# soedinglab/plass

Measured on AMD Instinct MI355X. Metric: read-overlaps/s per assembly iteration, higher is better.
Workload: dtype u8/u64 (integer hash, byte compare; f32 ratios)

## Files before the change

plass_amd/csrc/assemble.hip:

```cpp
#include "common.hpp"
#include "device_utils.hpp"
#include "posterior_class.hpp"
#include "host_util.hpp"
#include <algorithm>
#include <memory>
#include <cstring>

namespace plasship {

struct Item {
    uint32_t target; int32_t score; uint32_t alnLength; float seqId;
    int32_t qStart, qEnd; uint32_t qLen; int32_t dbStart, dbEnd; uint32_t dbLen;
    uint32_t state;
    uint32_t pad;
};

struct AsmArgs {
    SeqView s;
    const uint64_t *qoff; const AlnRec *recs;
    Item *items;
    const uint64_t *arenaOff;
    const uint32_t *leftCap;
    char *arena;
    uint32_t *flags;
    uint32_t *newLen;
    uint64_t *newStart;
    const signed char *mat;
    double lambda, logK, ln2;
    float seqIdThr; uint64_t maxSeqLen; int rescoreMode;
    uint32_t ownLaneMin;
    unsigned long long *stats;
    uint32_t *bigList; uint32_t nBig;
    uint32_t *midList; uint32_t nMid;
    uint32_t *mid32List; uint32_t nMid32;
    uint32_t *smallList; uint32_t nSmall;
    uint32_t *heap;
    const uint32_t *ambKeys; const uint8_t *ambVals; uint32_t ambMask;
    uint32_t *needKeys; uint32_t *needCount; uint32_t needCap;
    uint32_t *redoList; uint32_t *redoCount;
    const uint32_t *queryList; uint32_t nQueryList;
    uint8_t *cmpCache;
    SeqView aa; char *aaArena; const uint64_t *aaArenaOff; const uint32_t *aaLeftCap; uint32_t *aaNewLen; uint64_t *aaNewStart;
};

__device__ __forceinline__ float seqIdThroughText(float f) {
    if (f == 1.0f) return 1.0f;
    const int t = (int) (f * 1000);
    int zeros = 0;
    if ((double) f < 0.10) zeros++;
    if ((double) f < 0.01) zeros++;
    int digits = 1; for (int x = t; x >= 10; x /= 10) digits++;
    double den = 1.0; for (int i = 0; i < digits + zeros; i++) den *= 10.0;
    return (float) ((double) t / den);
}

__device__ __forceinline__ uint64_t loadU64Unaligned(const char *p) { uint64_t w; __builtin_memcpy(&w, p, 8); return w; }
__device__ __forceinline__ void storeU64Unaligned(char *p, uint64_t w) { __builtin_memcpy(p, &w, 8); }
__device__ __forceinline__ void storeTail(char *d, uint64_t v, unsigned r) {
    if (r & 4u) { const uint32_t x = (uint32_t) v; __builtin_memcpy(d, &x, 4); d += 4; v >>= 32; }
    if (r & 2u) { const uint16_t x = (uint16_t) v; __builtin_memcpy(d, &x, 2); d += 2; v >>= 16; }
    if (r & 1u) *d = (char) v;
}
template <int G> __device__ __forceinline__ void copyBytesG(char *dst, const char *src, unsigned n, int gl) {
    for (unsigned i = 8u * (unsigned) gl; i < n; i += 8u * G) {
        const uint64_t w = loadU64Unaligned(src + i);
        if (i + 8 <= n) storeU64Unaligned(dst + i, w);
        else storeTail(dst + i, w, n - i);
    }
}
__device__ __forceinline__ void stageScoreTable(signed char *smat, const signed char *__restrict__ mat, int nThreads) {
    for (int i = threadIdx.x; i < 123 * 123; i += nThreads) smat[i] = i ? mat[i] : (signed char) 0;
}
__device__ __forceinline__ uint64_t byteRangeMask(int lo, int hi) {
    const uint64_t belowHi = hi >= 8 ? ~0ULL : (hi <= 0 ? 0ULL : ((1ULL << (8 * hi)) - 1ULL));
    const uint64_t belowLo = lo >= 8 ? ~0ULL : (lo <= 0 ? 0ULL : ((1ULL << (8 * lo)) - 1ULL));
    return belowHi & ~belowLo;
}
__device__ __forceinline__ int zeroBytes(uint64_t x, uint64_t mask) {
    const uint64_t lo7 = 0x7F7F7F7F7F7F7F7FULL;
    return __popcll(~(((x & lo7) + lo7) | x | lo7) & mask);
}
template <int G> __device__ __forceinline__ void scoreColumnsG(const char *q, const char *t, unsigned len, const signed char *smat, int gl,
                                                               unsigned &first, unsigned &last, int &s, int &ids) {
    const unsigned p0 = 8u * (unsigned) gl;
    uint64_t qw = 0, tw = 0;
// ... 23 lines not shown
__device__ __forceinline__ void scoreColumnsSerial(const char *q, const char *t, unsigned len, const signed char *smat,
                                                   unsigned &first, unsigned &last, int &s, int &ids) {
    const char q0 = q[0], t0 = t[0], qe = q[len - 1], te = t[len - 1];
    uint64_t qw[4], tw[4];
    __builtin_memcpy(qw, q, 32); __builtin_memcpy(tw, t, 32);
    first = (q0 == '*' || t0 == '*') ? 1u : 0u;
    last = len - 1;
    if (last > 0 && (qe == '*' || te == '*')) last--;
    for (unsigned p = 0; p < len; p += 32) {
        if (p) { __builtin_memcpy(qw, q + p, 32); __builtin_memcpy(tw, t + p, 32); }
#pragma unroll
        for (unsigned k = 0; k < 4; k++) {
            const int lo = (int) first - (int) (p + 8 * k), hi = (int) last - (int) (p + 8 * k);
            uint64_t qv = qw[k], tv = tw[k];
            if (lo <= 0 && hi >= 8) ids += zeroBytes(qw[k] ^ tw[k], ~0ULL);
            else {
                const uint64_t m = byteRangeMask(lo, hi + 1);
                ids += zeroBytes(qw[k] ^ tw[k], byteRangeMask(lo, hi));
                qv = qw[k] & m; tv = tw[k] & m;
            }
#pragma unroll
            for (unsigned j = 0; j < 8; j++) {
                const unsigned a = (unsigned) (qv >> (8 * j)) & 0xFFu, b = (unsigned) (tv >> (8 * j)) & 0xFFu;
                s += (int) smat[a * 123 + b];
            }
        }
    }
}

struct Rescored { int startPos, endPos; unsigned score, diagonalLen; int idExcl; };
__device__ __forceinline__ Rescored rescoreOnDiagonal(const char *q, unsigned qLen, const char *t, unsigned tLen, int diagonal,
                                                      const signed char *smat) {
    Rescored r; r.startPos = -1; r.endPos = -1; r.score = 0; r.diagonalLen = 0; r.idExcl = 0;
    const unsigned dist = (unsigned) abs(diagonal);
    unsigned qo, to, len;
    if (diagonal >= 0 && dist < qLen) { qo = dist; to = 0; len = min(tLen, qLen - dist); }
    else if (diagonal < 0 && dist < tLen) { qo = 0; to = dist; len = min(tLen - dist, qLen); }
    else return r;
    r.diagonalLen = len;
    if (len == 0) return r;
    unsigned first, last;
    int s = 0, ids = 0;
    scoreColumnsG<64>(q + qo, t + to, len, smat, laneId(), first, last, s, ids);
    s = waveReduceSum(s); ids = waveReduceSum(ids);
    r.score = (unsigned) max(s, 0); r.startPos = (int) first; r.endPos = (int) last; r.idExcl = ids;
    return r;
}

__device__ __forceinline__ void waveMemSync() {
    __builtin_amdgcn_fence(__ATOMIC_RELEASE, "workgroup");
    __builtin_amdgcn_fence(__ATOMIC_ACQUIRE, "workgroup");
}
__global__ __launch_bounds__(256) void assembleBigKernel(AsmArgs a) {
    __shared__ signed char smat[123 * 123 + 7];
    stageScoreTable(smat, a.mat, 256);
    __syncthreads();
    const int lane = threadIdx.x & 63;
    unsigned long long nExt = 0, nResc = 0, nRescRes = 0, nAln = 0, nQRes = 0;
    for (uint32_t w = blockIdx.x * 4 + (threadIdx.x >> 6); w < a.nBig; w += gridDim.x * 4) {
        const uint32_t id = a.bigList[w];
        const uint64_t h0 = a.qoff[id], h1 = a.qoff[id + 1];
        const uint32_t h = (uint32_t) (h1 - h0);
        if (h == 0) continue;
        const uint64_t aoff = a.arenaOff[id];
        if (a.arenaOff[id + 1] == aoff) continue;
        Item *it = a.items + h0;
        const char *orig = a.s.data + seqOff(a.s, id);
        unsigned querySeqLen = seqLen(a.s, id);
        nAln += h; nQRes += querySeqLen;
        for (uint32_t i = lane; i < h; i += 64) {
            const AlnRec r = a.recs[h0 + i];
            Item x;
            x.target = r.target;
            const int aq = (r.qStart == -1) ? 0 : r.qStart, ad = (r.dbStart == -1) ? 0 : r.dbStart;
            x.alnLength = (uint32_t) (max(abs(r.qEnd - aq), abs(r.dbEnd - ad)) + 1);
            const int rawScore = (int) (fma((double) r.bitScore, a.ln2, a.logK) / a.lambda + 0.5);
            const float scorePerCol = (float) rawScore / (float) ((double) x.alnLength + 0.5);
            const float sid = r.fromText ? r.seqId : seqIdThroughText(r.seqId);
            const float alnLen = (float) x.alnLength;
            const float ids = sid * alnLen;
            x.seqId = (float) ((double) ids / ((double) alnLen + 0.5));
            x.score = (int) (scorePerCol * 100);
            x.qStart = r.qStart; x.qEnd = r.qEnd; x.qLen = (uint32_t) r.qLen; x.dbStart = r.dbStart; x.dbEnd = r.dbEnd; x.dbLen = (uint32_t) r.dbLen;
            x.state = r.accepted ? 0u : 2u; x.pad = 0;
            it[i] = x;
        }
        char *buf = a.arena + aoff;
        uint64_t curStart = a.leftCap[id];
        copyBytesG<64>(buf + curStart, orig, querySeqLen, lane);
        uint64_t curLen = querySeqLen;
        waveMemSync();
        bool couldExtend = false;
        uint32_t inQueue = h;
        while (inQueue > 0) {
            unsigned leftOff = 0, rightOff = 0;
            bool brokeOut = false;
            unsigned long long bestR = 0, bestL = 0; uint32_t idxR = 0xFFFFFFFFu, idxL = 0xFFFFFFFFu;
            for (uint32_t i = lane; i < h; i += 64) {
                Item x = it[i];
                if (x.state == 1) { it[i].state = 2; continue; }
                if (x.state != 0) continue;
                const unsigned long long key = ((unsigned long long) ((uint32_t) x.score ^ 0x80000000u) << 32) | (unsigned long long) x.alnLength;
                const bool notBoth = !(x.dbStart == 0 && x.qStart == 0);
                const bool rightStart = x.dbStart == 0 && (x.dbEnd != (int) x.dbLen - 1);
                const bool leftStart = x.qStart == 0 && (x.qEnd != (int) x.qLen - 1);
                if (!((rightStart || leftStart) && notBoth) || x.target == id) continue;
                const unsigned tLen = seqLen(a.s, x.target);
                if (x.dbStart == 0) {
                    const unsigned fragR = tLen - ((unsigned) x.dbEnd + 1);
                    if (fragR > 0 && (unsigned) x.qEnd == (querySeqLen - 1) && (key > bestR || (key == bestR && x.target < it[idxR].target))) { bestR = key; idxR = i; }
                } else if (x.qStart == 0) {
                    if (x.dbStart > 0 && (unsigned) x.dbEnd == (tLen - 1) && (key > bestL || (key == bestL && x.target < it[idxL].target))) { bestL = key; idxL = i; }
                }
            }
            uint32_t tgtR = idxR != 0xFFFFFFFFu ? it[idxR].target : 0xFFFFFFFFu, tgtL = idxL != 0xFFFFFFFFu ? it[idxL].target : 0xFFFFFFFFu;
#pragma unroll
            for (int o = 32; o > 0; o >>= 1) {
                const unsigned long long okR = __shfl_xor(bestR, o, 64), okL = __shfl_xor(bestL, o, 64);
                const uint32_t oiR = __shfl_xor(idxR, o, 64), oiL = __shfl_xor(idxL, o, 64), otR = __shfl_xor(tgtR, o, 64), otL = __shfl_xor(tgtL, o, 64);
                if (oiR != 0xFFFFFFFFu && (idxR == 0xFFFFFFFFu || okR > bestR || (okR == bestR && otR < tgtR))) { bestR = okR; idxR = oiR; tgtR = otR; }
                if (oiL != 0xFFFFFFFFu && (idxL == 0xFFFFFFFFu || okL > bestL || (okL == bestL && otL < tgtL))) { bestL = okL; idxL = oiL; tgtL = otL; }
            }
            const bool haveR = idxR != 0xFFFFFFFFu, haveL = idxL != 0xFFFFFFFFu;
            const bool rFirst = haveR && (!haveL || bestR > bestL || (bestR == bestL && tgtR < tgtL));
            waveMemSync();
            auto extendRight = [&]() {
                const Item x = it[idxR];
                const char *tSeq = a.s.data + seqOff(a.s, x.target);
                const unsigned tLen = seqLen(a.s, x.target), dbEnd = (unsigned) x.dbEnd, fragLen = tLen - (dbEnd + 1);
                copyBytesG<64>(buf + curStart + curLen, tSeq + dbEnd + 1, fragLen, lane);
                curLen += fragLen; rightOff += fragLen;
                if (lane == 0) atomicOr(&a.flags[x.target], 0x80u);
            };
            if (rFirst) extendRight();
            if (haveL) {
                const Item x = it[idxL];
                const unsigned fragLen = (unsigned) x.dbStart;
                if (curLen + fragLen >= a.maxSeqLen) brokeOut = true;
                else {
                    const char *tSeq = a.s.data + seqOff(a.s, x.target);
                    curStart -= fragLen;
                    copyBytesG<64>(buf + curStart, tSeq, fragLen, lane);
                    curLen += fragLen; leftOff += fragLen;
                    if (lane == 0) atomicOr(&a.flags[x.target], 0x80u);
                }
            }
            if (haveR && !rFirst && !brokeOut) extendRight();
            waveMemSync();
            uint32_t still = 0;
// ... 11 lines not shown
                const bool rightStart = x.dbStart == 0 && (x.dbEnd != (int) x.dbLen - 1);
                const bool leftStart = x.qStart == 0 && (x.qEnd != (int) x.qLen - 1);
                if (!used && (rightStart || leftStart) && notBoth && x.target != id) {
                    const unsigned tLen = seqLen(a.s, x.target);
                    if (x.dbStart == 0) { if ((tLen - ((unsigned) x.dbEnd + 1)) > rightOff && (unsigned) x.qEnd == (querySeqLen - 1) && rightOff > 0) st = 1; }
                    else if (x.qStart == 0) { if (x.dbStart > (int) leftOff && (unsigned) x.dbEnd == (tLen - 1) && leftOff > 0) st = 1; }
                }
                it[i].state = st;
            }
            inQueue = (uint32_t) waveReduceSum((int) still);
            waveMemSync();
            if (leftOff > 0 || rightOff > 0) couldExtend = true;
            if (brokeOut && inQueue > 0) break;
            querySeqLen = (unsigned) curLen;
            const char *qs = buf + curStart;
            waveMemSync();
            for (uint32_t i = lane; i < h; i += 64) {
                Item x = it[i];
                if (x.state != 1) continue;
                const char *tSeq = a.s.data + seqOff(a.s, x.target);
                const unsigned tLen = seqLen(a.s, x.target);
                const int diag = (int) ((unsigned) x.qStart + leftOff) - x.dbStart;
                const unsigned dist = (unsigned) abs(diag);
                unsigned qo = 0, to = 0, len = 0; bool hit = true;
                if (diag >= 0 && dist < querySeqLen) { qo = dist; to = 0; len = min(tLen, querySeqLen - dist); }
                else if (diag < 0 && dist < tLen) { qo = 0; to = dist; len = min(tLen - dist, querySeqLen); }
                else hit = false;
                unsigned first = 0, last = 0; int sc = 0, ids = 0; int startPos = -1, endPos = -1;
                if (hit && len > 0) { scoreColumnsSerial(qs + qo, tSeq + to, len, smat, first, last, sc, ids); startPos = (int) first; endPos = (int) last; }
                const unsigned score = (unsigned) max(sc, 0);
                nResc++; nRescRes += hit ? len : 0;
                int qS, qE, dS, dE;
                if (diag >= 0) { qS = startPos + (int) dist; qE = endPos + (int) dist; dS = startPos; dE = endPos; }
                else { qS = startPos; qE = endPos; dS = startPos + (int) dist; dE = endPos + (int) dist; }
                const float seqId = (float) ids / ((float) qE - (float) qS);
                x.seqId = seqId; x.qLen = querySeqLen; x.dbLen = tLen; x.alnLength = hit ? len : 0u;
                const float spc = (float) score / (float) ((double) x.alnLength + 0.5);
                x.score = (int) (spc * 100);
                x.qStart = qS; x.qEnd = qE; x.dbStart = dS; x.dbEnd = dE;
                x.state = (seqId >= a.seqIdThr) ? 0u : 2u;
                it[i] = x;
            }
            waveMemSync();
            {
                uint32_t c = 0;
                for (uint32_t i = lane; i < h; i += 64) c += (it[i].state == 0) ? 1u : 0u;
                inQueue = (uint32_t) waveReduceSum((int) c);
            }
        }
        if (couldExtend) {
            if (lane == 0) { atomicOr(&a.flags[id], 0x20u); a.newLen[id] = (uint32_t) curLen; a.newStart[id] = aoff + curStart; }
            nExt++;
        }
        waveMemSync();
    }
    nResc = waveReduceSumU64(nResc); nRescRes = waveReduceSumU64(nRescRes);
    if (lane == 0) {
        if (nExt) atomicAdd(&a.stats[0], nExt); if (nResc) atomicAdd(&a.stats[1], nResc); if (nRescRes) atomicAdd(&a.stats[2], nRescRes);
        if (nAln) { atomicAdd(&a.stats[9], nAln); atomicAdd(&a.stats[10], nQRes); atomicAdd(&a.stats[11], nRescRes); }
    }
}

__device__ __forceinline__ char nuclRevN(char c) {
    switch (c & ~0x20) {
        case 'A': return 'T';
        case 'C': case 'M': case 'Y': case 'H': return 'G';
        case 'T': case 'U': case 'W': return 'A';
        case 'G': case 'K': case 'B': case 'D': case 'V': case 'R': case 'S': return 'C';
        default: return 'N';
    }
}
constexpr unsigned CMP_LEN = 512, CMP_MM = 8;
struct NuclCmp { const AsmArgs *a; bool abort; };
__device__ __forceinline__ uint32_t ambHash(uint32_t a1, uint32_t b1, uint32_t a2, uint32_t b2) {
    return (a1 * 0x9E3779B1u) ^ (b1 * 0x85EBCA77u) ^ (a2 * 0xC2B2AE3Du) ^ (b2 * 0x27D4EB2Fu);
}
__device__ __attribute__((noinline)) int nuclPosteriorClassDev(unsigned alpha1, unsigned beta1, unsigned alpha2, unsigned beta2, const AsmArgs *ap) {
    const double p = nuclPosteriorP(alpha1, beta1, alpha2, beta2);
    int cls = (p < 0.45) ? 0 : ((p > 0.55) ? 1 : 2);
    const double AMB_EPS = nuclPosteriorBand(alpha1, beta1, alpha2, beta2);
    if (fabs(p - 0.45) < AMB_EPS || fabs(p - 0.55) < AMB_EPS) {
        const AsmArgs &a = *ap;
        if (a.ambMask) {
            uint32_t slot = ambHash(alpha1, beta1, alpha2, beta2) & a.ambMask;
            for (;;) {
                const uint32_t *k = a.ambKeys + 4 * (size_t) slot;
                if (k[0] == 0) break;
                if (k[0] == alpha1 && k[1] == beta1 && k[2] == alpha2 && k[3] == beta2) return (int) a.ambVals[slot];
                slot = (slot + 1) & a.ambMask;
            }
        }
        const uint32_t w = atomicAdd(a.needCount, 1u);
        if (w < a.needCap) { uint32_t *k = a.needKeys + 4 * (size_t) w; k[0] = alpha1; k[1] = beta1; k[2] = alpha2; k[3] = beta2; }
        return -1;
    }
    return cls;
}
__device__ __forceinline__ bool nuclLess(const Item &r1, const Item &r2, NuclCmp &c) {
    if (c.abort) return false;
    const unsigned mm1 = (unsigned) ((double) ((1.0f - r1.seqId) * (float) r1.alnLength) + 0.5);
    const unsigned mm2 = (unsigned) ((double) ((1.0f - r2.seqId) * (float) r2.alnLength) + 0.5);
    const bool cacheable = c.a->cmpCache && mm1 < CMP_MM && mm2 < CMP_MM && r1.alnLength < CMP_LEN && r2.alnLength < CMP_LEN;
    const size_t cidx = cacheable ? ((((size_t) r1.alnLength * CMP_MM + mm1) * CMP_LEN + r2.alnLength) * CMP_MM + mm2) : 0;
    int cls = cacheable ? (int) c.a->cmpCache[cidx] - 1 : -1;
    if (cls < 0) {
        cls = nuclPosteriorClassDev(mm1 + 1, r1.alnLength - mm1 + 1, mm2 + 1, r2.alnLength - mm2 + 1, c.a);
        if (cls < 0) { c.abort = true; return false; }
// ... 1132 lines not shown
    }
    const unsigned gridN = std::min<uint32_t>((N + 255) / 256 + 1, 8192);
    hipLaunchKernelGGL(extMarkKernel, dim3(gridN), dim3(256), 0, st, N, dFlags, dNewLen, guided ? dAaNewLen : (const uint32_t *) nullptr, dKeep.as<uint32_t>(), dBytes.as<uint64_t>(),
                       guided ? dAaBytes.as<uint64_t>() : (uint64_t *) nullptr);
    if (exclusiveScanU32(st, dKeep.as<uint32_t>(), dPos.as<uint64_t>(), N, dTmp, tmpBytes) || exclusiveScanU64(st, dBytes.as<uint64_t>(), dOff.as<uint64_t>(), N, dTmp, tmpBytes) ||
        (guided && exclusiveScanU64(st, dAaBytes.as<uint64_t>(), dAaOff.as<uint64_t>(), N, dTmp, tmpBytes))) { setError("plasship_assemble: scan failed"); return PLASSHIP_ERR_DEVICE; }
    uint64_t nExt = 0, extBytes = 0, aaExtBytes = 0;
    PH_CHECK(hipMemcpyAsync(&nExt, dPos.as<uint64_t>() + N, 8, hipMemcpyDeviceToHost, st));
    PH_CHECK(hipMemcpyAsync(&extBytes, dOff.as<uint64_t>() + N, 8, hipMemcpyDeviceToHost, st));
    if (guided) PH_CHECK(hipMemcpyAsync(&aaExtBytes, dAaOff.as<uint64_t>() + N, 8, hipMemcpyDeviceToHost, st));
    PH_CHECK(plasship::streamSync(st));
    DevBuf dMeta, dPacked, dAaPacked;
    if (dMeta.alloc(std::max<uint64_t>(nExt, 1) * sizeof(ExtMeta)) != hipSuccess || dPacked.alloc(extBytes + 64) != hipSuccess || (guided && dAaPacked.alloc(aaExtBytes + 64) != hipSuccess)) {
        setError("plasship_assemble: out of device memory"); return PLASSHIP_ERR_DEVICE;
    }
    if (N) hipLaunchKernelGGL(extPackKernel, dim3(std::min<uint32_t>((N + 15) / 16, (uint32_t) ctx->numCU * 16)), dim3(256), 0, st, N, dKeep.as<uint32_t>(), dPos.as<uint64_t>(), dOff.as<uint64_t>(),
                              guided ? dAaOff.as<uint64_t>() : (const uint64_t *) nullptr, dNewLen, dNewStart, dArena, dAaNewLen, dAaNewStart, dAaArena,
                              dMeta.as<ExtMeta>(), dPacked.as<char>(), guided ? dAaPacked.as<char>() : (char *) nullptr);
    PH_TRACE(st, "assemble: packed the extended sequences");
    DevBuf gMeta; std::vector<uint64_t> rb(W), rbMeta(W), rbSeq(W), rbAa(W);
    uint64_t M = 0;
    {
        const uint64_t mine[3] = {nExt, extBytes, aaExtBytes}; std::vector<uint64_t> all(3 * (size_t) W);
        const int rc0 = commAllgatherHost(ctx, mine, all.data(), 24); if (rc0) return rc0;
        for (int r = 0; r < W; r++) { M += all[3 * (size_t) r]; rbMeta[r] = all[3 * (size_t) r] * sizeof(ExtMeta); rbSeq[r] = all[3 * (size_t) r + 1]; rbAa[r] = all[3 * (size_t) r + 2]; }
    }
    int rc = commAllgathervBytesKnown(ctx, dMeta.p, nExt * sizeof(ExtMeta), gMeta, rbMeta); if (rc) return rc;
    rc = commAllgathervBytesKnown(ctx, dPacked.p, extBytes, gathered, rbSeq); if (rc) return rc;
    if (guided) { rc = commAllgathervBytesKnown(ctx, dAaPacked.p, aaExtBytes, gatheredAa, rbAa); if (rc) return rc; }
    PH_TRACE(st, "assemble: gathered the extended sequences");
    DevBuf dLens, dStart, dAaLens, dAaStart, dTmp2; const size_t tmp2Bytes = exclusiveScanTmpBytes(M + 2);
    if (dLens.alloc((M + 1) * 8) != hipSuccess || dStart.alloc((M + 2) * 8) != hipSuccess || dTmp2.alloc(tmp2Bytes) != hipSuccess ||
        (guided && (dAaLens.alloc((M + 1) * 8) != hipSuccess || dAaStart.alloc((M + 2) * 8) != hipSuccess))) { setError("plasship_assemble: out of device memory"); return PLASSHIP_ERR_DEVICE; }
    if (M) {
        const unsigned gridM = (unsigned) std::min<uint64_t>((M + 255) / 256, 8192);
        hipLaunchKernelGGL(extLensKernel, dim3(gridM), dim3(256), 0, st, gMeta.as<ExtMeta>(), M, dLens.as<uint64_t>(), guided ? dAaLens.as<uint64_t>() : (uint64_t *) nullptr);
        if (exclusiveScanU64(st, dLens.as<uint64_t>(), dStart.as<uint64_t>(), M, dTmp2.p, tmp2Bytes) ||
            (guided && exclusiveScanU64(st, dAaLens.as<uint64_t>(), dAaStart.as<uint64_t>(), M, dTmp2.p, tmp2Bytes))) { setError("plasship_assemble: scan failed"); return PLASSHIP_ERR_DEVICE; }
        hipLaunchKernelGGL(extMergeKernel, dim3(gridM), dim3(256), 0, st, gMeta.as<ExtMeta>(), M, dStart.as<uint64_t>(), guided ? dAaStart.as<uint64_t>() : (const uint64_t *) nullptr,
                           dFlags, dNewLen, dNewStart, dAaNewLen, dAaNewStart);
    }
    PH_TRACE(st, "assemble: merged the extended sequences");
    if (!keepTarget) {
        DevBuf gFlags;
        rc = commAllgathervBytes(ctx, dFlags, (uint64_t) N * 4, gFlags, rb); if (rc) return rc;
        if (N) hipLaunchKernelGGL(orFlagsKernel, dim3(gridN), dim3(256), 0, st, gFlags.as<uint32_t>(), N, W, dFlags);
        PH_CHECK(plasship::streamSync(st));
    }
    PH_CHECK(plasship::streamSync(st));
    PH_CHECK(hipGetLastError());
    return PLASSHIP_OK;
}

static int assembleImpl(plasship_ctx *ctx, const plasship_seqdb *db, const plasship_seqdb *aaDb, const plasship_alns *al,
                        const plasship_assemble_params *par, plasship_seqdb **out, plasship_seqdb **outAa, plasship_assemble_stats *stats) {
    const bool guided = aaDb != nullptr;
    const bool nucl = db->dbtype == PLASSHIP_DBTYPE_NUCLEOTIDES;
    if (!nucl && db->dbtype != PLASSHIP_DBTYPE_AMINO_ACIDS) { setError("plasship_assemble: the sequence DB is neither amino acids nor nucleotides"); return PLASSHIP_ERR_ARG; }
    if (par->rescore_mode != 3) { setError("plasship_assemble: only --rescore-mode 3"); return PLASSHIP_ERR_UNSUPPORTED; }
    if (al->nQueries != db->n) { setError("plasship_assemble: alignment list does not belong to the DB"); return PLASSHIP_ERR_ARG; }
    PH_ENTER(ctx);
    hipStream_t st = ctx->stream;
    const uint32_t N = (uint32_t) db->n;
    if (nucl) { const int rcS = finishSelfAlns(ctx, al); if (rcS) return rcS; }
    const uint64_t nLines = al->nSlots;
    DevBuf dLeftCap, dBytes, dArenaOff, dTmp, dItems, dFlags, dNewLen, dNewStart, dMat, dStats, dArena;
    const size_t tmpBytes = exclusiveScanTmpBytes((size_t) N + 2);
    if (dLeftCap.alloc(((size_t) N + 1) * 4) != hipSuccess || dBytes.alloc(((size_t) N + 1) * 8) != hipSuccess || dArenaOff.alloc(((size_t) N + 2) * 8) != hipSuccess ||
        dTmp.alloc(tmpBytes) != hipSuccess || dItems.alloc(std::max<uint64_t>(nLines, 1) * sizeof(Item)) != hipSuccess || dFlags.alloc(((size_t) N + 1) * 4) != hipSuccess ||
        dNewLen.alloc(((size_t) N + 1) * 4) != hipSuccess || dNewStart.alloc(((size_t) N + 1) * 8) != hipSuccess || dMat.alloc(123 * 123) != hipSuccess || dStats.alloc(128) != hipSuccess) {
        setError("plasship_assemble: out of device memory"); return PLASSHIP_ERR_DEVICE;
    }
    PH_CHECK(hipMemsetAsync(dFlags.p, 0, ((size_t) N + 1) * 4, st));
    PH_CHECK(hipMemsetAsync(dNewLen.p, 0, ((size_t) N + 1) * 4, st));
    PH_CHECK(hipMemsetAsync(dStats.p, 0, 128, st));
    PH_CHECK(hipMemcpyAsync(dMat.p, asciiSubMat(nucl), 123 * 123, hipMemcpyHostToDevice, st));
    { const int rcOL = ensureOffLen(ctx, db); if (rcOL) return rcOL; }
    const SeqView sv = db->view();
    PH_CHECK(hipEventRecord(ctx->ev[0], st));
    DevBuf dBigList, dMidList, dMid32List, dSmallList, dTierA, dTierB, dPosA, dPosB, dAaLeftCap, dAaBytes, dAaArenaOff, dAaArena, dAaNewLen, dAaNewStart;
    if (guided && (dAaLeftCap.alloc(((size_t) N + 1) * 4) != hipSuccess || dAaBytes.alloc(((size_t) N + 1) * 8) != hipSuccess || dAaArenaOff.alloc(((size_t) N + 2) * 8) != hipSuccess ||
                   dAaNewLen.alloc(((size_t) N + 1) * 4) != hipSuccess || dAaNewStart.alloc(((size_t) N + 1) * 8) != hipSuccess)) { setError("plasship_assemble: out of device memory"); return PLASSHIP_ERR_DEVICE; }
    if (guided) PH_CHECK(hipMemsetAsync(dAaNewLen.p, 0, ((size_t) N + 1) * 4, st));
    if (dBigList.alloc(((size_t) N + 1) * 4) != hipSuccess || dMidList.alloc(((size_t) N + 1) * 4) != hipSuccess || dMid32List.alloc(((size_t) N + 1) * 4) != hipSuccess ||
        dSmallList.alloc(((size_t) N + 1) * 4) != hipSuccess || dTierA.alloc(((size_t) N + 1) * 8) != hipSuccess || dTierB.alloc(((size_t) N + 1) * 8) != hipSuccess ||
        dPosA.alloc(((size_t) N + 2) * 8) != hipSuccess || dPosB.alloc(((size_t) N + 2) * 8) != hipSuccess) { setError("plasship_assemble: out of device memory"); return PLASSHIP_ERR_DEVICE; }
    DevBuf dQSum, dQSumAa, dQCan;
    if (dQSum.alloc(((size_t) N + 1) * 8) != hipSuccess || dQCan.alloc(((size_t) N + 1) * 4) != hipSuccess || (guided && dQSumAa.alloc(((size_t) N + 1) * 8) != hipSuccess)) { setError("plasship_assemble: out of device memory"); return PLASSHIP_ERR_DEVICE; }
    PH_CHECK(hipMemsetAsync(dQSum.p, 0, ((size_t) N + 1) * 8, st));
    PH_CHECK(hipMemsetAsync(dQCan.p, 0, ((size_t) N + 1) * 4, st));
    if (guided) PH_CHECK(hipMemsetAsync(dQSumAa.p, 0, ((size_t) N + 1) * 8, st));
    if (nLines) hipLaunchKernelGGL(arenaSumKernel, dim3((unsigned) std::min<uint64_t>((nLines + 255) / 256, (uint64_t) ctx->numCU * 32)), dim3(256), 0, st, al->d_recs.as<AlnRec>(), (uint64_t) nLines,
                                       (uint64_t) par->max_seq_len, dQSum.as<unsigned long long>(), guided ? dQSumAa.as<unsigned long long>() : (unsigned long long *) nullptr, dQCan.as<uint32_t>(),
                                       (nucl && !guided) ? 1 : 0);
    if (N) hipLaunchKernelGGL(arenaSizeKernel, dim3(std::min<uint32_t>((N + 255) / 256, 8192)), dim3(256), 0, st, sv, al->d_qoff.as<uint64_t>(), (const unsigned long long *) dQSum.as<unsigned long long>(),
                              (const unsigned long long *) dQSumAa.as<unsigned long long>(), (const uint32_t *) dQCan.as<uint32_t>(), dLeftCap.as<uint32_t>(), dBytes.as<uint64_t>(), nucl ? 1 : 0, (uint64_t) tuneInt("NUCL_THREAD_BYTES", 1 << 30),
                              dTierA.as<uint64_t>(), dTierB.as<uint64_t>(),
                              guided ? aaDb->d_len.as<uint32_t>() : (const uint32_t *) nullptr, dAaLeftCap.as<uint32_t>(), guided ? dAaBytes.as<uint64_t>() : (uint64_t *) nullptr);
    if (guided && exclusiveScanU64(st, dAaBytes.as<uint64_t>(), dAaArenaOff.as<uint64_t>(), N, dTmp.p, tmpBytes)) { setError("plasship_assemble: scan failed"); return PLASSHIP_ERR_DEVICE; }
    if (exclusiveScanU64(st, dTierA.as<uint64_t>(), dPosA.as<uint64_t>(), N, dTmp.p, tmpBytes) || exclusiveScanU64(st, dTierB.as<uint64_t>(), dPosB.as<uint64_t>(), N, dTmp.p, tmpBytes)) {
        setError("plasship_assemble: scan failed"); return PLASSHIP_ERR_DEVICE;
    }
    if (N) hipLaunchKernelGGL(listKernel, dim3(std::min<uint32_t>((N + 255) / 256, 8192)), dim3(256), 0, st, N, dTierA.as<uint64_t>(), dTierB.as<uint64_t>(), dPosA.as<uint64_t>(), dPosB.as<uint64_t>(),
                              dSmallList.as<uint32_t>(), dMid32List.as<uint32_t>(), dMidList.as<uint32_t>(), dBigList.as<uint32_t>());
    if (exclusiveScanU64(st, dBytes.as<uint64_t>(), dArenaOff.as<uint64_t>(), N, dTmp.p, tmpBytes)) { setError("plasship_assemble: scan failed"); return PLASSHIP_ERR_DEVICE; }
    uint64_t arenaBytes = 0, aaArenaBytes = 0;
// ... 58 lines not shown
                if (cnts[0]) {
                    a.queryList = dSmallList.as<uint32_t>(); a.nQueryList = cnts[0];
                    if (tuneInt("NUCL_CLASSES", 1) == 1) {
                        DevBuf dCls;
                        if (dCls.alloc(2 * NW_CLASSES * 4) != hipSuccess) { setError("plasship_assemble: out of device memory"); return PLASSHIP_ERR_DEVICE; }
                        PH_CHECK(hipMemsetAsync(dCls.p, 0, 2 * NW_CLASSES * 4, st));
                        const unsigned g = std::min<uint32_t>((cnts[0] + 255) / 256, (uint32_t) ctx->numCU * 8);
                        hipLaunchKernelGGL(nuclClassCountKernel, dim3(g), dim3(256), 0, st, (const uint32_t *) dSmallList.as<uint32_t>(), cnts[0], (const uint64_t *) dBytes.as<uint64_t>(), dCls.as<uint32_t>());
                        hipLaunchKernelGGL(nuclClassScatterKernel, dim3(g), dim3(256), 0, st, (const uint32_t *) dSmallList.as<uint32_t>(), cnts[0], (const uint64_t *) dBytes.as<uint64_t>(), dCls.as<uint32_t>(),
                                           dMidList.as<uint32_t>());
                        a.queryList = dMidList.as<uint32_t>();
                    }
                    const uint32_t grid = std::min<uint32_t>((cnts[0] + NT_BLOCK - 1) / NT_BLOCK, (uint32_t) ctx->numCU * 8);
                    if (guided) hipLaunchKernelGGL(assembleNuclThreadKernel<true>, dim3(grid), dim3(NT_BLOCK), 0, st, a);
                    else hipLaunchKernelGGL(assembleNuclThreadKernel<false>, dim3(grid), dim3(NT_BLOCK), 0, st, a);
                }
                launchWave(dMid32List.as<uint32_t>(), cnts[1]);
            } else launchWave(dRedo[(pass + 1) & 1].as<uint32_t>(), nWork);
            uint32_t cnt[2] = {0, 0};
            PH_CHECK(hipMemcpyAsync(cnt, dCnt.p, 8, hipMemcpyDeviceToHost, st));
            PH_CHECK(plasship::streamSync(st));
            PH_CHECK(hipGetLastError());
            nWork = cnt[1];
            if (nWork == 0) break;
            const uint32_t nNeed = std::min(cnt[0], needCap);
            if (nNeed == 0) { setError("plasship_assemble: queries aborted without a missing comparator tuple"); return PLASSHIP_ERR_DEVICE; }
            std::vector<uint32_t> need((size_t) nNeed * 4);
            PH_COPY_SYNC(ctx->stream, need.data(), dNeed.p, need.size() * 4, hipMemcpyDeviceToHost);
            const int rc = ambTableInsert(ctx, need.data(), nNeed);
            if (rc != PLASSHIP_OK) return rc;
        }
        PH_CHECK(hipEventRecord(ctx->ev[3], st));
        for (int e = 4; e <= 7; e++) PH_CHECK(hipEventRecord(ctx->ev[e], st));
    } else {
    const int w16 = tuneInt("ASM16", 5), w64 = tuneInt("ASM64", 4);
    const uint32_t gx = (uint32_t) std::max(1, tuneInt("ASM_GRIDX", 1));
    const dim3 g16(std::min<uint32_t>((a.nSmall + 15) / 16, (uint32_t) ctx->numCU * (uint32_t) w16 * gx)), g64(std::min<uint32_t>((a.nMid + 3) / 4, (uint32_t) ctx->numCU * (uint32_t) w64 * gx));
    PH_CHECK(hipEventRecord(ctx->ev[2], st));
    if (a.nSmall) {
        if (w16 == 6) hipLaunchKernelGGL((assembleGroupKernel<16, 6>), g16, dim3(256), 0, st, a);
        else if (w16 == 5) hipLaunchKernelGGL((assembleGroupKernel<16, 5>), g16, dim3(256), 0, st, a);
        else hipLaunchKernelGGL((assembleGroupKernel<16, 4>), g16, dim3(256), 0, st, a);
    }
    PH_CHECK(hipEventRecord(ctx->ev[3], st));
    PH_CHECK(hipEventRecord(ctx->ev[4], st));
    if (a.nMid32) hipLaunchKernelGGL((assembleGroupKernel<32, 5>), dim3(std::min<uint32_t>((a.nMid32 + 7) / 8, (uint32_t) ctx->numCU * 5u * gx)), dim3(256), 0, st, a);
    if (a.nMid) {
        if (w64 == 5) hipLaunchKernelGGL((assembleGroupKernel<64, 5>), g64, dim3(256), 0, st, a);
        else if (w64 == 4) hipLaunchKernelGGL((assembleGroupKernel<64, 4>), g64, dim3(256), 0, st, a);
        else hipLaunchKernelGGL((assembleGroupKernel<64, 3>), g64, dim3(256), 0, st, a);
    }
    PH_CHECK(hipEventRecord(ctx->ev[5], st));
    PH_CHECK(hipEventRecord(ctx->ev[6], st));
    if (a.nBig) hipLaunchKernelGGL(assembleBigKernel, dim3(std::min<uint32_t>((a.nBig + 3) / 4, (uint32_t) ctx->numCU * (uint32_t) tuneInt("ASMBIG", 4))), dim3(256), 0, st, a);
    PH_CHECK(hipEventRecord(ctx->ev[7], st));
    }
    PH_TRACE(st, "assemble: extension kernels");
    plasship_seqdb *o = nullptr, *oAa = nullptr;
    unsigned long long hs[16] = {0};
    DevBuf dGathered, dGatheredAa;
    const char *arenaP = dArena.as<char>(), *aaArenaP = dAaArena.as<char>();
    if (commOf(ctx)) {
        const int rc = mergeExtended(ctx, N, guided, par->keep_target, dFlags.as<uint32_t>(), dNewLen.as<uint32_t>(), dNewStart.as<uint64_t>(), dArena.as<char>(),
                                     dAaNewLen.as<uint32_t>(), dAaNewStart.as<uint64_t>(), dAaArena.as<char>(), dTmp.p, tmpBytes, dGathered, dGatheredAa);
        if (rc != PLASSHIP_OK) return rc;
        arenaP = dGathered.as<char>(); aaArenaP = dGatheredAa.as<char>();
    }
    int rcOut = buildOutputDB(ctx, db, dFlags.as<uint32_t>(), dNewLen.as<uint32_t>(), dNewStart.as<uint64_t>(), arenaP, par->keep_target, dTmp.p, tmpBytes, &o,
                              dStats.p, hs, 128, guided ? (hipEvent_t) nullptr : ctx->ev[1], guided);
    if (rcOut != PLASSHIP_OK) return rcOut;
    std::unique_ptr<plasship_seqdb> holdO(o), holdAa;
    if (guided) {
        rcOut = buildOutputDB(ctx, aaDb, dFlags.as<uint32_t>(), dAaNewLen.as<uint32_t>(), dAaNewStart.as<uint64_t>(), aaArenaP, par->keep_target, dTmp.p, tmpBytes, &oAa,
                              nullptr, nullptr, 0, nullptr, true);
        if (rcOut != PLASSHIP_OK) return rcOut;
        holdAa.reset(oAa);
    }
    if (guided) { PH_CHECK(hipEventRecord(ctx->ev[1], st)); PH_CHECK(plasship::streamSync(st)); }
    if (hs[12]) { setError("plasship_guided_assemble: an alignment asks for a protein fragment the twin does not have (coordinates are not codon aligned)"); return PLASSHIP_ERR_ARG; }
    if (stats) {
        stats->n_extended = hs[0]; stats->n_rescored = hs[1]; stats->out_residues = o->residues;
        float ms = 0; (void) hipEventElapsedTime(&ms, ctx->ev[0], ctx->ev[1]); stats->ms_kernel = ms;
        float sum = 0;
        for (int t = 0; t < 3; t++) {
            ms = 0; (void) hipEventElapsedTime(&ms, ctx->ev[2 + 2 * t], ctx->ev[3 + 2 * t]); stats->ms_tier_kernel[t] = ms; sum += ms;
            stats->tier_alignments[t] = hs[3 + 3 * t]; stats->tier_query_residues[t] = hs[4 + 3 * t]; stats->tier_rescored_residues[t] = hs[5 + 3 * t];
        }
        stats->ms_assemble_kernel = sum;
        stats->n_alignments = al->nLines; stats->rescored_residues = hs[2];
        stats->db_appended_bytes = o->buildAppendedBytes; stats->db_copied_bytes = o->buildCopiedBytes;
    }
    *out = holdO.release();
    if (guided) *outAa = holdAa.release();
    return PLASSHIP_OK;
}

extern "C" int plasship_assemble(plasship_ctx *ctx, const plasship_seqdb *db, const plasship_alns *al,
                                 const plasship_assemble_params *par, plasship_seqdb **out, plasship_assemble_stats *stats) {
    if (!ctx || !db || !al || !par || !out) { setError("plasship_assemble: bad argument"); return PLASSHIP_ERR_ARG; }
    return commFinish(ctx, assembleImpl(ctx, db, nullptr, al, par, out, nullptr, stats));
}

extern "C" int plasship_guided_assemble(plasship_ctx *ctx, const plasship_seqdb *nucl_db, const plasship_seqdb *aa_db, const plasship_alns *al,
                                        const plasship_assemble_params *par, plasship_seqdb **out_nucl, plasship_seqdb **out_aa,
                                        plasship_assemble_stats *stats) {
    if (!ctx || !nucl_db || !aa_db || !al || !par || !out_nucl || !out_aa) { setError("plasship_guided_assemble: bad argument"); return PLASSHIP_ERR_ARG; }
    if (nucl_db->dbtype != PLASSHIP_DBTYPE_NUCLEOTIDES || aa_db->dbtype != PLASSHIP_DBTYPE_AMINO_ACIDS) { setError("plasship_guided_assemble: needs a nucleotide DB and its protein twin DB"); return PLASSHIP_ERR_ARG; }
    if (nucl_db->n != aa_db->n) { setError("plasship_guided_assemble: the two DBs differ in size"); return PLASSHIP_ERR_ARG; }
// ... 7 lines not shown
```

Baseline: 707.4 million.

## Add LDS-resident compacting queue kernels for big-query assembly with overflow fallback

```diff
diff --git a/plass_amd/csrc/assemble.hip b/plass_amd/csrc/assemble.hip
--- a/plass_amd/csrc/assemble.hip
+++ b/plass_amd/csrc/assemble.hip
@@ -31,6 +31,10 @@
     uint32_t ownLaneMin;
     unsigned long long *stats;
     uint32_t *bigList; uint32_t nBig;
+    const uint32_t *bigCount;
+    uint32_t *overList; uint32_t *overCount;
+    uint32_t queueCap;
+    uint32_t *dbgRounds; uint32_t *dbgCycles;
     uint32_t *midList; uint32_t nMid;
     uint32_t *mid32List; uint32_t nMid32;
     uint32_t *smallList; uint32_t nSmall;
@@ -160,12 +164,14 @@
     __builtin_amdgcn_fence(__ATOMIC_ACQUIRE, "workgroup");
 }
 __global__ __launch_bounds__(256) void assembleBigKernel(AsmArgs a) {
+    const uint32_t nBig = a.bigCount ? *a.bigCount : a.nBig;
+    if (blockIdx.x * 4 >= nBig) return;
     __shared__ signed char smat[123 * 123 + 7];
     stageScoreTable(smat, a.mat, 256);
     __syncthreads();
     const int lane = threadIdx.x & 63;
     unsigned long long nExt = 0, nResc = 0, nRescRes = 0, nAln = 0, nQRes = 0;
-    for (uint32_t w = blockIdx.x * 4 + (threadIdx.x >> 6); w < a.nBig; w += gridDim.x * 4) {
+    for (uint32_t w = blockIdx.x * 4 + (threadIdx.x >> 6); w < nBig; w += gridDim.x * 4) {
         const uint32_t id = a.bigList[w];
         const uint64_t h0 = a.qoff[id], h1 = a.qoff[id + 1];
         const uint32_t h = (uint32_t) (h1 - h0);
@@ -176,6 +182,7 @@
         const char *orig = a.s.data + seqOff(a.s, id);
         unsigned querySeqLen = seqLen(a.s, id);
         nAln += h; nQRes += querySeqLen;
+        const uint64_t t0 = a.dbgRounds ? (uint64_t) clock64() : 0; uint32_t rounds = 0;
         for (uint32_t i = lane; i < h; i += 64) {
             const AlnRec r = a.recs[h0 + i];
             Item x;
@@ -203,6 +210,7 @@
         while (inQueue > 0) {
             unsigned leftOff = 0, rightOff = 0;
             bool brokeOut = false;
+            rounds++;
             unsigned long long bestR = 0, bestL = 0; uint32_t idxR = 0xFFFFFFFFu, idxL = 0xFFFFFFFFu;
             for (uint32_t i = lane; i < h; i += 64) {
                 Item x = it[i];
@@ -320,7 +328,213 @@
             if (lane == 0) { atomicOr(&a.flags[id], 0x20u); a.newLen[id] = (uint32_t) curLen; a.newStart[id] = aoff + curStart; }
             nExt++;
         }
+        if (a.dbgRounds && lane == 0) { a.dbgRounds[id] = rounds | (couldExtend ? 0x80000000u : 0u); a.dbgCycles[id] = (uint32_t) min<uint64_t>((uint64_t) clock64() - t0, 0xFFFFFFFFull); }
         waveMemSync();
+    }
+    nResc = waveReduceSumU64(nResc); nRescRes = waveReduceSumU64(nRescRes);
+    if (lane == 0) {
+        if (nExt) atomicAdd(&a.stats[0], nExt); if (nResc) atomicAdd(&a.stats[1], nResc); if (nRescRes) atomicAdd(&a.stats[2], nRescRes);
+        if (nAln) { atomicAdd(&a.stats[9], nAln); atomicAdd(&a.stats[10], nQRes); atomicAdd(&a.stats[11], nRescRes); }
+    }
+}
+
+constexpr uint32_t ASMQ_CAP1 = 128, ASMQ_CAP = 256;
+template <int CAP> struct QueueLds {
+    unsigned long long key[CAP];
+    uint64_t offLen[CAP];
+    uint32_t target[CAP], qLen[CAP], dbLen[CAP];
+    int32_t qStart[CAP], qEnd[CAP], dbStart[CAP], dbEnd[CAP];
+};
+struct QItem { unsigned long long key; uint64_t offLen; uint32_t target, qLen, dbLen; int32_t qStart, qEnd, dbStart, dbEnd; };
+template <int CAP> __device__ __forceinline__ QItem qLoad(const QueueLds<CAP> &q, uint32_t i) {
+    QItem x;
+    x.key = q.key[i]; x.offLen = q.offLen[i]; x.target = q.target[i]; x.qLen = q.qLen[i]; x.dbLen = q.dbLen[i];
+    x.qStart = q.qStart[i]; x.qEnd = q.qEnd[i]; x.dbStart = q.dbStart[i]; x.dbEnd = q.dbEnd[i];
+    return x;
+}
+template <int CAP> __device__ __forceinline__ void qStore(QueueLds<CAP> &q, uint32_t i, const QItem &x) {
+    q.key[i] = x.key; q.offLen[i] = x.offLen; q.target[i] = x.target; q.qLen[i] = x.qLen; q.dbLen[i] = x.dbLen;
+    q.qStart[i] = x.qStart; q.qEnd[i] = x.qEnd; q.dbStart[i] = x.dbStart; q.dbEnd[i] = x.dbEnd;
+}
+template <int CAP> __device__ __forceinline__ uint32_t qCompact(QueueLds<CAP> &q, uint32_t base, bool keep, const QItem &x) {
+    const unsigned long long m = __ballot(keep);
+    if (keep) qStore(q, base + (uint32_t) __builtin_amdgcn_mbcnt_hi((uint32_t) (m >> 32), __builtin_amdgcn_mbcnt_lo((uint32_t) m, 0u)), x);
+    return (uint32_t) __popcll(m);
+}
+__device__ __forceinline__ void queueFence() { __builtin_amdgcn_fence(__ATOMIC_ACQ_REL, "wavefront"); __builtin_amdgcn_wave_barrier(); }
+__device__ __forceinline__ unsigned long long queueKey(int score, uint32_t alnLength) {
+    return ((unsigned long long) ((uint32_t) score ^ 0x80000000u) << 32) | (unsigned long long) alnLength;
+}
+
+template <int CAP, int WPE>
+__global__ __launch_bounds__(256) __attribute__((amdgpu_waves_per_eu(WPE, WPE))) void assembleQueueKernel(AsmArgs a) {
+    const uint32_t nBig = a.bigCount ? *a.bigCount : a.nBig;
+    if (blockIdx.x * 4 >= nBig) return;
+    __shared__ signed char smat[123 * 123 + 7];
+    __shared__ QueueLds<CAP> queues[4];
+    stageScoreTable(smat, a.mat, 256);
+    __syncthreads();
+    const int lane = threadIdx.x & 63;
+    QueueLds<CAP> &q = queues[threadIdx.x >> 6];
+    unsigned long long nExt = 0, nResc = 0, nRescRes = 0, nAln = 0, nQRes = 0;
+    for (uint32_t w = blockIdx.x * 4 + (threadIdx.x >> 6); w < nBig; w += gridDim.x * 4) {
+        const uint32_t id = a.bigList[w];
+        const uint64_t h0 = a.qoff[id], h1 = a.qoff[id + 1];
+        const uint32_t h = (uint32_t) (h1 - h0);
+        if (h == 0) continue;
+        if (h > CAP || h > a.queueCap) {
+            if (lane == 0) a.overList[atomicAdd(a.overCount, 1u)] = id;
+            continue;
+        }
+        const uint64_t aoff = a.arenaOff[id];
+        if (a.arenaOff[id + 1] == aoff) continue;
+        const uint64_t qOffLen = a.s.offLen[id];
+        const char *orig = a.s.data + (qOffLen >> 24);
+        unsigned querySeqLen = (unsigned) ((uint32_t) qOffLen & 0xFFFFFFu);
+        nAln += h; nQRes += querySeqLen;
+        const uint64_t t0 = a.dbgRounds ? (uint64_t) clock64() : 0; uint32_t rounds = 0;
+        uint32_t n = 0;
+        for (uint32_t b = 0; b < h; b += 64) {
+            const uint32_t i = b + (uint32_t) lane;
+            QItem x; bool keep = false;
+            if (i < h) {
+                const AlnRec r = a.recs[h0 + i];
+                x.target = r.target;
+                const int aq = (r.qStart == -1) ? 0 : r.qStart, ad = (r.dbStart == -1) ? 0 : r.dbStart;
+                const uint32_t alnLength = (uint32_t) (max(abs(r.qEnd - aq), abs(r.dbEnd - ad)) + 1);
+                const int rawScore = (int) (fma((double) r.bitScore, a.ln2, a.logK) / a.lambda + 0.5);
+                const float scorePerCol = (float) rawScore / (float) ((double) alnLength + 0.5);
+                x.key = queueKey((int) (scorePerCol * 100), alnLength);
+                x.qStart = r.qStart; x.qEnd = r.qEnd; x.qLen = (uint32_t) r.qLen; x.dbStart = r.dbStart; x.dbEnd = r.dbEnd; x.dbLen = (uint32_t) r.dbLen;
+                keep = r.accepted != 0;
+                const bool branchType = ((x.dbStart == 0 && x.dbEnd != (int) x.dbLen - 1) || (x.qStart == 0 && x.qEnd != (int) x.qLen - 1)) && !(x.dbStart == 0 && x.qStart == 0);
+                x.offLen = (keep && branchType && x.target != id) ? a.s.offLen[x.target] : 0;
+            }
+            n += qCompact(q, n, keep, x);
+        }
+        queueFence();
+        char *buf = a.arena + aoff;
+        uint64_t curStart = a.leftCap[id];
+        copyBytesG<64>(buf + curStart, orig, querySeqLen, lane);
+        uint64_t curLen = querySeqLen;
+        bool couldExtend = false;
+        while (n > 0) {
+            unsigned leftOff = 0, rightOff = 0;
+            bool brokeOut = false;
+            rounds++;
+            unsigned long long bestR = 0, bestL = 0; uint32_t idxR = 0xFFFFFFFFu, idxL = 0xFFFFFFFFu, tgtR = 0xFFFFFFFFu, tgtL = 0xFFFFFFFFu;
+            for (uint32_t i = lane; i < n; i += 64) {
+                const QItem x = qLoad(q, i);
+                const bool notBoth = !(x.dbStart == 0 && x.qStart == 0);
+                const bool rightStart = x.dbStart == 0 && (x.dbEnd != (int) x.dbLen - 1);
+                const bool leftStart = x.qStart == 0 && (x.qEnd != (int) x.qLen - 1);
+                if (!((rightStart || leftStart) && notBoth) || x.target == id) continue;
+                const unsigned tLen = (uint32_t) x.offLen & 0xFFFFFFu;
+                if (x.dbStart == 0) {
+                    const unsigned fragR = tLen - ((unsigned) x.dbEnd + 1);
+                    if (fragR > 0 && (unsigned) x.qEnd == (querySeqLen - 1) && (x.key > bestR || (x.key == bestR && x.target < tgtR))) { bestR = x.key; idxR = i; tgtR = x.target; }
+                } else if (x.qStart == 0) {
+                    if (x.dbStart > 0 && (unsigned) x.dbEnd == (tLen - 1) && (x.key > bestL || (x.key == bestL && x.target < tgtL))) { bestL = x.key; idxL = i; tgtL = x.target; }
+                }
+            }
+#pragma unroll
+            for (int o = 32; o > 0; o >>= 1) {
+                const unsigned long long okR = __shfl_xor(bestR, o, 64), okL = __shfl_xor(bestL, o, 64);
+                const uint32_t oiR = __shfl_xor(idxR, o, 64), oiL = __shfl_xor(idxL, o, 64), otR = __shfl_xor(tgtR, o, 64), otL = __shfl_xor(tgtL, o, 64);
+                if (oiR != 0xFFFFFFFFu && (idxR == 0xFFFFFFFFu || okR > bestR || (okR == bestR && otR < tgtR))) { bestR = okR; idxR = oiR; tgtR = otR; }
+                if (oiL != 0xFFFFFFFFu && (idxL == 0xFFFFFFFFu || okL > bestL || (okL == bestL && otL < tgtL))) { bestL = okL; idxL = oiL; tgtL = otL; }
+            }
+            const bool haveR = idxR != 0xFFFFFFFFu, haveL = idxL != 0xFFFFFFFFu;
+            const bool rFirst = haveR && (!haveL || bestR > bestL || (bestR == bestL && tgtR < tgtL));
+            auto extendRight = [&]() {
+                const uint64_t ol = q.offLen[idxR];
+                const unsigned tLen = (uint32_t) ol & 0xFFFFFFu, dbEnd = (unsigned) q.dbEnd[idxR], fragLen = tLen - (dbEnd + 1);
+                copyBytesG<64>(buf + curStart + curLen, a.s.data + (ol >> 24) + dbEnd + 1, fragLen, lane);
+                curLen += fragLen; rightOff += fragLen;
+                if (lane == 0) atomicOr(&a.flags[tgtR], 0x80u);
+            };
+            if (rFirst) extendRight();
+            if (haveL) {
+                const unsigned fragLen = (unsigned) q.dbStart[idxL];
+                if (curLen + fragLen >= a.maxSeqLen) brokeOut = true;
+                else {
+                    curStart -= fragLen;
+                    copyBytesG<64>(buf + curStart, a.s.data + (q.offLen[idxL] >> 24), fragLen, lane);
+                    curLen += fragLen; leftOff += fragLen;
+                    if (lane == 0) atomicOr(&a.flags[tgtL], 0x80u);
+                }
+            }
+            if (haveR && !rFirst && !brokeOut) extendRight();
+            if (leftOff > 0 || rightOff > 0) couldExtend = true;
+            queueFence();
+            if (brokeOut) {
+                uint32_t still = 0;
+                for (uint32_t i = lane; i < n; i += 64) {
+                    const unsigned long long key = q.key[i];
+                    still += (key < bestL || (key == bestL && q.target[i] > tgtL)) ? 1u : 0u;
+                }
+                if (waveReduceSum((int) still) > 0) break;
+            }
+            uint32_t nd = 0;
+            for (uint32_t b = 0; b < n; b += 64) {
+                const uint32_t i = b + (uint32_t) lane;
+                QItem x; bool deferred = false;
+                if (i < n) {
+                    x = qLoad(q, i);
+                    const bool used = (i == idxR && (rFirst || !brokeOut)) || i == idxL;
+                    const bool notBoth = !(x.dbStart == 0 && x.qStart == 0);
+                    const bool rightStart = x.dbStart == 0 && (x.dbEnd != (int) x.dbLen - 1);
+                    const bool leftStart = x.qStart == 0 && (x.qEnd != (int) x.qLen - 1);
+                    if (!used && (rightStart || leftStart) && notBoth && x.target != id) {
+                        const unsigned tLen = (uint32_t) x.offLen & 0xFFFFFFu;
+                        if (x.dbStart == 0) deferred = (tLen - ((unsigned) x.dbEnd + 1)) > rightOff && (unsigned) x.qEnd == (querySeqLen - 1) && rightOff > 0;
+                        else if (x.qStart == 0) deferred = x.dbStart > (int) leftOff && (unsigned) x.dbEnd == (tLen - 1) && leftOff > 0;
+                    }
+                }
+                nd += qCompact(q, nd, deferred, x);
+            }
+            queueFence();
+            querySeqLen = (unsigned) curLen;
+            const char *qs = buf + curStart;
+            if (nd) waveMemSync();
+            uint32_t nn = 0;
+            for (uint32_t b = 0; b < nd; b += 64) {
+                const uint32_t i = b + (uint32_t) lane;
+                QItem x; bool keep = false;
+                if (i < nd) {
+                    x = qLoad(q, i);
+                    const char *tSeq = a.s.data + (x.offLen >> 24);
+                    const unsigned tLen = (uint32_t) x.offLen & 0xFFFFFFu;
+                    const int diag = (int) ((unsigned) x.qStart + leftOff) - x.dbStart;
+                    const unsigned dist = (unsigned) abs(diag);
+                    unsigned qo = 0, to = 0, len = 0; bool hit = true;
+                    if (diag >= 0 && dist < querySeqLen) { qo = dist; to = 0; len = min(tLen, querySeqLen - dist); }
+                    else if (diag < 0 && dist < tLen) { qo = 0; to = dist; len = min(tLen - dist, querySeqLen); }
+                    else hit = false;
+                    unsigned first = 0, last = 0; int sc = 0, ids = 0; int startPos = -1, endPos = -1;
+                    if (hit && len > 0) { scoreColumnsSerial(qs + qo, tSeq + to, len, smat, first, last, sc, ids); startPos = (int) first; endPos = (int) last; }
+                    const unsigned score = (unsigned) max(sc, 0);
+                    nResc++; nRescRes += hit ? len : 0;
+                    int qS, qE, dS, dE;
+                    if (diag >= 0) { qS = startPos + (int) dist; qE = endPos + (int) dist; dS = startPos; dE = endPos; }
+                    else { qS = startPos; qE = endPos; dS = startPos + (int) dist; dE = endPos + (int) dist; }
+                    const float seqId = (float) ids / ((float) qE - (float) qS);
+                    const uint32_t alnLength = hit ? len : 0u;
+                    const float spc = (float) score / (float) ((double) alnLength + 0.5);
+                    x.key = queueKey((int) (spc * 100), alnLength); x.qLen = querySeqLen; x.dbLen = tLen;
+                    x.qStart = qS; x.qEnd = qE; x.dbStart = dS; x.dbEnd = dE;
+                    keep = seqId >= a.seqIdThr;
+                }
+                nn += qCompact(q, nn, keep, x);
+            }
+            queueFence();
+            n = nn;
+        }
+        if (couldExtend) {
+            if (lane == 0) { atomicOr(&a.flags[id], 0x20u); a.newLen[id] = (uint32_t) curLen; a.newStart[id] = aoff + curStart; }
+            nExt++;
+        }
+        if (a.dbgRounds && lane == 0) { a.dbgRounds[id] = rounds | (couldExtend ? 0x80000000u : 0u); a.dbgCycles[id] = (uint32_t) min<uint64_t>((uint64_t) clock64() - t0, 0xFFFFFFFFull); }
     }
     nResc = waveReduceSumU64(nResc); nRescRes = waveReduceSumU64(nRescRes);
     if (lane == 0) {
@@ -1559,6 +1773,39 @@
     return PLASSHIP_OK;
 }
 
+static bool asmHistOn() { return getenv("PLASSHIP_DEBUG_ASMHIST") != nullptr; }
+static int asmHistRecord(hipStream_t st, uint32_t N, const uint64_t *dQoff, const uint32_t *dBigList, uint32_t nBig, const uint32_t *dRounds, const uint32_t *dCycles,
+                         uint32_t cap) {
+    static int call = 0;
+    std::vector<uint32_t> ids(nBig), rounds(N), cycles(N);
+    std::vector<uint64_t> qoff((size_t) N + 1);
+    if (nBig) PH_COPY_SYNC(st, ids.data(), dBigList, (size_t) nBig * 4, hipMemcpyDeviceToHost);
+    PH_COPY_SYNC(st, qoff.data(), dQoff, ((size_t) N + 1) * 8, hipMemcpyDeviceToHost);
+    PH_COPY_SYNC(st, rounds.data(), dRounds, (size_t) N * 4, hipMemcpyDeviceToHost);
+    PH_COPY_SYNC(st, cycles.data(), dCycles, (size_t) N * 4, hipMemcpyDeviceToHost);
+    constexpr int NH = 5, NR = 8;
+    uint64_t hq[NH] = {}, hx[NH] = {}, hr[NH] = {}, hc[NH] = {}, hm[NH] = {}, rq[NR] = {}, ct = 0, over = 0, maxH = 0;
+    for (uint32_t w = 0; w < nBig; w++) {
+        const uint32_t id = ids[w], h = (uint32_t) (qoff[id + 1] - qoff[id]), r = rounds[id] & 0x7FFFFFFFu;
+        int b = 0; while (b < NH - 1 && h > (128u << b)) b++;
+        int k = 0; if (r) { k = 1; uint32_t e = 1; while (k < NR - 1 && r > e) { e <<= 1; k++; } }
+        hq[b]++; hx[b] += rounds[id] >> 31; hr[b] += r; hm[b] = std::max<uint64_t>(hm[b], r); hc[b] += cycles[id]; ct += cycles[id];
+        rq[k]++; over += h > cap; maxH = std::max<uint64_t>(maxH, h);
+    }
+    std::string s = "asmHist call " + std::to_string(call++) + " big queries " + std::to_string(nBig) + " (max h " + std::to_string(maxH) + ", over cap " +
+                    std::to_string(cap) + ": " + std::to_string(over) + ") | h bins <=128,<=256,<=512,<=1024,more: queries/extended/mean rounds/max rounds/% ticks";
+    for (int b = 0; b < NH; b++) {
+        char t[96];
+        snprintf(t, sizeof(t), " [%llu %llu %.2f %llu %.1f%%]", (unsigned long long) hq[b], (unsigned long long) hx[b], hq[b] ? (double) hr[b] / hq[b] : 0.0,
+                 (unsigned long long) hm[b], ct ? 100.0 * hc[b] / ct : 0.0);
+        s += t;
+    }
+    s += " | rounds 0,1,2,<=4,<=8,<=16,<=32,more:";
+    for (int k = 0; k < NR; k++) s += " " + std::to_string(rq[k]);
+    fprintf(stderr, "%s\n", s.c_str());
+    return PLASSHIP_OK;
+}
+
 static int assembleImpl(plasship_ctx *ctx, const plasship_seqdb *db, const plasship_seqdb *aaDb, const plasship_alns *al,
                         const plasship_assemble_params *par, plasship_seqdb **out, plasship_seqdb **outAa, plasship_assemble_stats *stats) {
     const bool guided = aaDb != nullptr;
@@ -1723,8 +1970,32 @@
     }
     PH_CHECK(hipEventRecord(ctx->ev[5], st));
     PH_CHECK(hipEventRecord(ctx->ev[6], st));
-    if (a.nBig) hipLaunchKernelGGL(assembleBigKernel, dim3(std::min<uint32_t>((a.nBig + 3) / 4, (uint32_t) ctx->numCU * (uint32_t) tuneInt("ASMBIG", 4))), dim3(256), 0, st, a);
+    DevBuf dDbgRounds, dDbgCycles;
+    const bool hist = asmHistOn() && a.nBig;
+    if (hist) {
+        if (dDbgRounds.alloc(((size_t) N + 1) * 4) != hipSuccess || dDbgCycles.alloc(((size_t) N + 1) * 4) != hipSuccess) { setError("plasship_assemble: out of device memory"); return PLASSHIP_ERR_DEVICE; }
+        PH_CHECK(hipMemsetAsync(dDbgRounds.p, 0, ((size_t) N + 1) * 4, st));
+        PH_CHECK(hipMemsetAsync(dDbgCycles.p, 0, ((size_t) N + 1) * 4, st));
+        a.dbgRounds = dDbgRounds.as<uint32_t>(); a.dbgCycles = dDbgCycles.as<uint32_t>();
+    }
+    const bool onChip = tuneInt("ASMQ", 1) != 2;
+    const uint32_t qCap = (uint32_t) std::max(0, std::min(tuneInt("ASMQ_CAP", (int) ASMQ_CAP), (int) ASMQ_CAP));
+    const dim3 gBig(std::min<uint32_t>((a.nBig + 3) / 4, (uint32_t) ctx->numCU * (uint32_t) tuneInt("ASMBIG", 4)));
+    DevBuf dOverList[2], dOverCount;
+    if (a.nBig && onChip) {
+        if (dOverList[0].alloc(((size_t) a.nBig + 1) * 4) != hipSuccess || dOverList[1].alloc(((size_t) a.nBig + 1) * 4) != hipSuccess || dOverCount.alloc(8) != hipSuccess) {
+            setError("plasship_assemble: out of device memory"); return PLASSHIP_ERR_DEVICE;
+        }
+        PH_CHECK(hipMemsetAsync(dOverCount.p, 0, 8, st));
+        AsmArgs q1 = a; q1.overList = dOverList[0].as<uint32_t>(); q1.overCount = dOverCount.as<uint32_t>(); q1.queueCap = qCap;
+        hipLaunchKernelGGL((assembleQueueKernel<ASMQ_CAP1, 4>), dim3(std::min<uint32_t>((a.nBig + 3) / 4, (uint32_t) ctx->numCU * 4u)), dim3(256), 0, st, q1);
+        AsmArgs q2 = q1; q2.bigList = dOverList[0].as<uint32_t>(); q2.bigCount = dOverCount.as<uint32_t>(); q2.overList = dOverList[1].as<uint32_t>(); q2.overCount = dOverCount.as<uint32_t>() + 1;
+        hipLaunchKernelGGL((assembleQueueKernel<ASMQ_CAP, 2>), dim3(std::min<uint32_t>((a.nBig + 3) / 4, (uint32_t) ctx->numCU * 2u)), dim3(256), 0, st, q2);
+        AsmArgs o = a; o.bigList = dOverList[1].as<uint32_t>(); o.bigCount = dOverCount.as<uint32_t>() + 1;
+        hipLaunchKernelGGL(assembleBigKernel, gBig, dim3(256), 0, st, o);
+    } else if (a.nBig) hipLaunchKernelGGL(assembleBigKernel, gBig, dim3(256), 0, st, a);
     PH_CHECK(hipEventRecord(ctx->ev[7], st));
+    if (hist) { const int rcH = asmHistRecord(st, N, a.qoff, a.bigList, a.nBig, a.dbgRounds, a.dbgCycles, onChip ? qCap : 64); if (rcH) return rcH; }
     }
     PH_TRACE(st, "assemble: extension kernels");
     plasship_seqdb *o = nullptr, *oAa = nullptr;
```

Measured after the change: 720.1 million, median of 6. 1.8% higher.
